# mormj/newsched

Measured on NVIDIA B200. Metric: Msamples/s FIR-ccf & FFT-4096 flowgraph at 1/2/4/8 B200; % of HBM/FP32 roofline, higher is better.
Workload: dtype f32

## Files before the change

newsched_b200/csrc/fft.cu:

```cuda
#include <cmath>
#include <cstdlib>
#include <vector>

#include "fft_core.cuh"

#ifndef B200_FFT_TW2
#define B200_FFT_TW2 1
#endif
#ifndef B200_FFT_SHFL
#define B200_FFT_SHFL 0
#endif
#ifndef B200_FFT_LATEBAR
#define B200_FFT_LATEBAR 0
#endif

namespace b200 {

template <bool FWD, int OUT>
__global__ void __launch_bounds__(256, 2)
    fft4096_kernel(const float2* __restrict__ in, void* __restrict__ out, long long n_vec,
                   const float* __restrict__ weff, const float2* __restrict__ tw1,
                   const float2* __restrict__ tw2)
{
    __shared__ float2 sA[16 * F4K_STRIDE];
    __shared__ float2 sT2[256];
    const int tid = threadIdx.x;

    float wreg[16];
    float2 t1[16];
#pragma unroll
    for (int i = 0; i < 16; i++) {
        wreg[i] = __ldg(weff + i * 256 + tid);
        t1[i] = __ldg(tw1 + i * 256 + tid);
    }
    sT2[tid] = __ldg(tw2 + tid);
    __syncthreads();

    for (long long vec = blockIdx.x; vec < n_vec; vec += gridDim.x) {
        const float2* x = in + vec * 4096;
        float2 v[16];
        if (tid == 0 && vec + gridDim.x < n_vec && ((uintptr_t)in % 16 == 0))
            asm volatile("cp.async.bulk.prefetch.L2.global [%0], %1;" ::"l"(in + (vec + gridDim.x) * 4096),
                         "r"(4096 * 8)
                         : "memory");
#pragma unroll
        for (int i = 0; i < 16; i++)
            v[i] = __ldcs(x + i * 256 + tid);
#pragma unroll
        for (int i = 0; i < 16; i++)
            v[i] = __fmul2_rn(v[i], make_float2(wreg[i], wreg[i]));
        dft16<FWD>(v);
#pragma unroll
        for (int k0 = 0; k0 < 16; k0++)
            sA[k0 * F4K_STRIDE + tid] = cmul(v[pos16(k0)], t1[k0]);
        __syncthreads();
        {
            const int k0 = tid >> 4, n0 = tid & 15;
            float2* row = sA + k0 * F4K_STRIDE + n0;
#pragma unroll
            for (int i = 0; i < 16; i++)
                v[i] = row[i * 16];
            dft16<FWD>(v);
            row[0] = v[pos16(0)];
#pragma unroll
            for (int k1 = 1; k1 < 16; k1++)
                row[k1 * 16] = cmul(v[pos16(k1)], sT2[k1 * 16 + n0]);
        }
        __syncthreads();
        {
            const int k0 = tid & 15, k1 = tid >> 4;
            const float2* row = sA + k0 * F4K_STRIDE + k1 * 16;
#pragma unroll
            for (int i = 0; i < 16; i++)
                v[i] = row[i];
            dft16<FWD>(v);
            if (OUT == B200_FFT_OUT_COMPLEX) {
                float2* y = reinterpret_cast<float2*>(out) + vec * 4096;
#pragma unroll
                for (int k2 = 0; k2 < 16; k2++)
                    __stcs(y + k2 * 256 + tid, v[pos16(k2)]);
            } else {
                float* y = reinterpret_cast<float*>(out) + vec * 4096;
#pragma unroll
                for (int k2 = 0; k2 < 16; k2++) {
                    float2 z = v[pos16(k2)];
                    float p = fmaf(z.x, z.x, z.y * z.y);
                    __stcs(y + k2 * 256 + tid, OUT == B200_FFT_OUT_MAG ? sqrt_approx(p) : p);
                }
            }
        }
        __syncthreads();
    }
}

#ifndef B200_FFT_DBUF
#define B200_FFT_DBUF 0
#endif
#ifndef F4K_NBUF_MAG
#define F4K_NBUF_MAG 2
#endif
constexpr int f4k_nbuf(int out) { return out == B200_FFT_OUT_COMPLEX ? 1 : F4K_NBUF_MAG; }
constexpr size_t f4k_tma_smem(int out)
{
    return (size_t)f4k_nbuf(out) * 4096 * 8 + (B200_FFT_DBUF ? 2 : 1) * 16 * F4K_STRIDE * 8 + 256 * 8 + 32;
}

template <bool FWD, int OUT>
__global__ void __launch_bounds__(256, 2)
    fft4096_tma_kernel(const float2* __restrict__ in, void* __restrict__ out, long long n_vec,
                       const float* __restrict__ weff, const float2* __restrict__ tw1,
                       const float2* __restrict__ tw2)
{
    constexpr int NBUF = f4k_nbuf(OUT);
    extern __shared__ __align__(128) unsigned char smem_raw[];
    float2* sIn0 = reinterpret_cast<float2*>(smem_raw);
    float2* sA0 = sIn0 + 4096 * NBUF;
#if B200_FFT_DBUF
    float2* sT2 = sA0 + 2 * 16 * F4K_STRIDE;
#else
    float2* sT2 = sA0 + 16 * F4K_STRIDE;
#endif
    uint64_t* bar0 = reinterpret_cast<uint64_t*>(sT2 + 256);
    const int tid = threadIdx.x;

    if (tid == 0) {
#pragma unroll
        for (int i = 0; i < NBUF; i++)
            mbar_init(bar0 + i, 1);
        fence_mbar_init();
    }
    float wreg[16];
    float2 t1[16];
#pragma unroll
    for (int i = 0; i < 16; i++) {
        wreg[i] = __ldg(weff + i * 256 + tid);
        t1[i] = __ldg(tw1 + i * 256 + tid);
    }
    sT2[tid] = __ldg(tw2 + tid);
    __syncthreads();
#if B200_FFT_TW2 == 1
    float2 t2r[16];
#pragma unroll
    for (int k1 = 1; k1 < 16; k1++)
        t2r[k1] = sT2[k1 * 16 + (tid & 15)];
#endif
    pdl_wait();
    pdl_launch_dependents();
    long long vec = blockIdx.x;
    if (tid == 0) {
#pragma unroll
        for (int i = 0; i < NBUF; i++)
            if (vec + (long long)i * gridDim.x < n_vec) {
                mbar_arrive_expect_tx(bar0 + i, 4096 * 8);
                bulk_copy_g2s(sIn0 + 4096 * i, in + (vec + (long long)i * gridDim.x) * 4096, 4096 * 8, bar0 + i);
            }
    }
    uint32_t phase = 0;
    int it = 0;
    for (; vec < n_vec; vec += gridDim.x, it++) {
        float2 v[16];
        float2* sIn = sIn0 + (NBUF == 2 ? (it & 1) * 4096 : 0);
        uint64_t* bar = bar0 + (NBUF == 2 ? (it & 1) : 0);
        const uint32_t par = NBUF == 2 ? (uint32_t)((it >> 1) & 1) : phase;
#if B200_FFT_DBUF
        float2* sA = sA0 + (phase ? 16 * F4K_STRIDE : 0);
#else
        float2* sA = sA0;
#endif
        mbar_wait(bar, par);
        phase ^= 1;
#pragma unroll
        for (int i = 0; i < 16; i++)
            v[i] = sIn[i * 256 + tid];
#pragma unroll
        for (int i = 0; i < 16; i++)
            v[i] = __fmul2_rn(v[i], make_float2(wreg[i], wreg[i]));
        dft16<FWD>(v);
#if B200_FFT_LATEBAR
        __syncthreads();
#endif
#pragma unroll
        for (int k0 = 0; k0 < 16; k0++)
            sA[k0 * F4K_STRIDE + tid] = cmul(v[pos16(k0)], t1[k0]);
#if B200_FFT_TW2 == 2
        float2 t2r[16];
#pragma unroll
        for (int k1 = 1; k1 < 16; k1++)
            t2r[k1] = sT2[k1 * 16 + (tid & 15)];
#endif
        __syncthreads();
        if (tid == 0 && vec + (long long)NBUF * gridDim.x < n_vec) {
            mbar_arrive_expect_tx(bar, 4096 * 8);
            bulk_copy_g2s(sIn, in + (vec + (long long)NBUF * gridDim.x) * 4096, 4096 * 8, bar);
        }
#if B200_FFT_SHFL
        {
            const int k0 = tid >> 4, n0 = tid & 15;
            const float2* row = sA + k0 * F4K_STRIDE + n0;
#pragma unroll
            for (int i = 0; i < 16; i++)
                v[i] = row[i * 16];
            dft16<FWD>(v);
            float2 w[16];
            w[0] = v[pos16(0)];
#pragma unroll
            for (int k1 = 1; k1 < 16; k1++)
                w[k1] = cmul(v[pos16(k1)], t2r[k1]);
#pragma unroll
            for (int sft = 1; sft < 16; sft <<= 1) {
                const bool up = (n0 & sft) != 0;
#pragma unroll
                for (int i = 0; i < 16; i++) {
                    if (i & sft)
                        continue;
                    const float2 send = up ? w[i] : w[i | sft];
                    float2 recv;
                    recv.x = __shfl_xor_sync(0xffffffffu, send.x, sft);
                    recv.y = __shfl_xor_sync(0xffffffffu, send.y, sft);
                    if (up)
                        w[i] = recv;
                    else
                        w[i | sft] = recv;
                }
            }
#pragma unroll
            for (int i = 0; i < 16; i++)
                v[i] = w[i];
            dft16<FWD>(v);
            const int k1 = n0;
            if (OUT == B200_FFT_OUT_COMPLEX) {
                float2* y = reinterpret_cast<float2*>(out) + vec * 4096;
#pragma unroll
                for (int k2 = 0; k2 < 16; k2++)
                    __stcs(y + k2 * 256 + k1 * 16 + k0, v[pos16(k2)]);
            } else {
                float* y = reinterpret_cast<float*>(out) + vec * 4096;
#pragma unroll
                for (int k2 = 0; k2 < 16; k2++) {
                    float2 z = v[pos16(k2)];
                    float p = fmaf(z.x, z.x, z.y * z.y);
                    __stcs(y + k2 * 256 + k1 * 16 + k0, OUT == B200_FFT_OUT_MAG ? sqrt_approx(p) : p);
                }
            }
        }
#else
        {
            const int k0 = tid >> 4, n0 = tid & 15;
            float2* row = sA + k0 * F4K_STRIDE + n0;
#pragma unroll
            for (int i = 0; i < 16; i++)
                v[i] = row[i * 16];
            dft16<FWD>(v);
            row[0] = v[pos16(0)];
#pragma unroll
            for (int k1 = 1; k1 < 16; k1++)
#if B200_FFT_TW2
                row[k1 * 16] = cmul(v[pos16(k1)], t2r[k1]);
#else
                row[k1 * 16] = cmul(v[pos16(k1)], sT2[k1 * 16 + n0]);
#endif
        }
        __syncthreads();
        {
            const int k0 = tid & 15, k1 = tid >> 4;
            const float2* row = sA + k0 * F4K_STRIDE + k1 * 16;
#pragma unroll
            for (int i = 0; i < 16; i++)
                v[i] = row[i];
            dft16<FWD>(v);
            if (OUT == B200_FFT_OUT_COMPLEX) {
                float2* y = reinterpret_cast<float2*>(out) + vec * 4096;
#pragma unroll
                for (int k2 = 0; k2 < 16; k2++)
                    __stcs(y + k2 * 256 + tid, v[pos16(k2)]);
            } else {
                float* y = reinterpret_cast<float*>(out) + vec * 4096;
#pragma unroll
                for (int k2 = 0; k2 < 16; k2++) {
                    float2 z = v[pos16(k2)];
                    float p = fmaf(z.x, z.x, z.y * z.y);
                    __stcs(y + k2 * 256 + tid, OUT == B200_FFT_OUT_MAG ? sqrt_approx(p) : p);
                }
            }
        }
#endif
#if !B200_FFT_LATEBAR && !B200_FFT_DBUF
        __syncthreads();
#endif
    }
}

#ifndef B200_F8K_EARLY
#define B200_F8K_EARLY 0
#endif
constexpr size_t F8K_SMEM = 8192 * 8 + 16 * F4K_STRIDE * 8 + 256 * 8 + 32;

template <bool FWD, int I>
__device__ __forceinline__ float2 mul_w32(float2 z)
{
    constexpr double kPi = 3.14159265358979323846;
    constexpr float cr[16] = { 1.f, 0.98078528040323043f, 0.92387953251128674f, 0.83146961230254524f,
                               0.70710678118654752f, 0.55557023301960218f, 0.38268343236508977f,
                               0.19509032201612825f, 0.f, -0.19509032201612825f, -0.38268343236508977f,
                               -0.55557023301960218f, -0.70710678118654752f, -0.83146961230254524f,
                               -0.92387953251128674f, -0.98078528040323043f };
    constexpr float si[16] = { 0.f, 0.19509032201612825f, 0.38268343236508977f, 0.55557023301960218f,
                               0.70710678118654752f, 0.83146961230254524f, 0.92387953251128674f,
                               0.98078528040323043f, 1.f, 0.98078528040323043f, 0.92387953251128674f,
                               0.83146961230254524f, 0.70710678118654752f, 0.55557023301960218f,
                               0.38268343236508977f, 0.19509032201612825f };
    (void)kPi;
    if (I == 0)
        return z;
    constexpr float wr = cr[I], wi = FWD ? -si[I] : si[I];
    return make_float2(fmaf(-z.y, wi, z.x * wr), fmaf(z.x, wi, z.y * wr));
}

template <bool FWD, int I = 0>
__device__ __forceinline__ void f8k_split(float2 (&a)[16], float2* sIn, const float* __restrict__ w0,
                                          const float* __restrict__ w1, float2 wt, int tid)
{
    if constexpr (I < 16) {
        const float2 x0 = __fmul2_rn(sIn[I * 256 + tid], make_float2(w0[I], w0[I]));
        const float2 x1 = __fmul2_rn(sIn[4096 + I * 256 + tid], make_float2(w1[I], w1[I]));
        a[I] = x0 + x1;
        sIn[I * 256 + tid] = cmul(mul_w32<FWD, I>(x0 - x1), wt);
        f8k_split<FWD, I + 1>(a, sIn, w0, w1, wt, tid);
    }
}

template <bool FWD, int OUT>
__global__ void __launch_bounds__(256, 2)
    fft8192_kernel(const float2* __restrict__ in, void* __restrict__ out, long long n_vec,
                   const float* __restrict__ weff, const float2* __restrict__ tw1,
                   const float2* __restrict__ tw2, float odd_sign)
{
    extern __shared__ __align__(128) unsigned char smem_raw[];
    float2* sIn = reinterpret_cast<float2*>(smem_raw);
    float2* sA = sIn + 8192;
    float2* sT2 = sA + 16 * F4K_STRIDE;
    uint64_t* bar = reinterpret_cast<uint64_t*>(sT2 + 256);
    const int tid = threadIdx.x;
    if (tid == 0) {
        mbar_init(bar, 1);
        mbar_init(bar + 1, 1);
        fence_mbar_init();
    }
    float2 t1[16];
#pragma unroll
    for (int i = 0; i < 16; i++)
        t1[i] = __ldg(tw1 + i * 256 + tid);
    sT2[tid] = __ldg(tw2 + tid);
    float2 wt;
    {
        float sn, cs_;
        sincospif((float)tid / 4096.0f, &sn, &cs_);
        wt = make_float2(cs_ * odd_sign, (FWD ? -sn : sn) * odd_sign);
    }
    __syncthreads();
    pdl_wait();
    pdl_launch_dependents();
    long long vec = blockIdx.x;
    if (tid == 0 && vec < n_vec) {
        mbar_arrive_expect_tx(bar, 4096 * 8);
        bulk_copy_g2s(sIn, in + vec * 8192, 4096 * 8, bar);
        mbar_arrive_expect_tx(bar + 1, 4096 * 8);
        bulk_copy_g2s(sIn + 4096, in + vec * 8192 + 4096, 4096 * 8, bar + 1);
    }
    uint32_t phase = 0;
    for (; vec < n_vec; vec += gridDim.x) {
        float2 e[16], v[16];
// ... 436 lines not shown
            __stcs(dst, make_float4(m[0], m[1], m[2], m[3]));
            __stcs(dst + 1, make_float4(m[4], m[5], m[6], m[7]));
        }
    }
}

template <bool FWD, int OUT>
__global__ void __launch_bounds__(512)
    fft_generic_kernel(const float2* __restrict__ in, void* __restrict__ out, long long n_vec, int N,
                       int log2n, int vpb, const float* __restrict__ weff,
                       const float2* __restrict__ tw, float2 post, int flip)
{
    extern __shared__ __align__(16) float2 sbuf[];
    const int per_cta = vpb * N;
    float2* bx = sbuf;
    float2* by = sbuf + per_cta;
    const long long v0 = (long long)blockIdx.x * vpb;
    const int nv = (int)((n_vec - v0) < vpb ? (n_vec - v0) : vpb);
    if (nv <= 0)
        return;
    const int tot = nv * N;
    const float2* x = in + v0 * N;
    for (int i = threadIdx.x; i < tot; i += blockDim.x) {
        float2 t = __ldcs(x + i);
        float w = __ldg(weff + (i & (N - 1)));
        bx[i] = make_float2(t.x * w, t.y * w);
    }
    __syncthreads();
    const int half = N >> 1;
    int s_log = 0;
    for (int n_log = log2n; n_log >= 1; n_log--, s_log++) {
        const int m = 1 << (n_log - 1);
        const int s = 1 << s_log;
        for (int i = threadIdx.x; i < nv * half; i += blockDim.x) {
            int vi = i / half;
            int bi = i - vi * half;
            int p = bi >> s_log;
            int q = bi & (s - 1);
            const float2* xb = bx + vi * N;
            float2* yb = by + vi * N;
            float2 a = xb[q + s * p];
            float2 b = xb[q + s * (p + m)];
            float2 w = __ldg(tw + (p << (log2n - n_log)));
            float2 d = a - b;
            yb[q + s * 2 * p] = a + b;
            yb[q + s * (2 * p + 1)] = cmul(d, w);
        }
        __syncthreads();
        float2* t = bx;
        bx = by;
        by = t;
    }
    for (int i = threadIdx.x; i < tot; i += blockDim.x) {
        float2 z = bx[i];
        int k = i & (N - 1);
        if (OUT == B200_FFT_OUT_COMPLEX) {
            z = cmul(z, post);
            if (flip && (k & 1))
                z = make_float2(-z.x, -z.y);
            __stcs(reinterpret_cast<float2*>(out) + v0 * N + i, z);
        } else {
            float pw = fmaf(z.x, z.x, z.y * z.y);
            __stcs(reinterpret_cast<float*>(out) + v0 * N + i,
                   OUT == B200_FFT_OUT_MAG ? sqrt_approx(pw) : pw);
        }
    }
}

}

using namespace b200;

struct b200_fft {
    int N = 0, log2n = 0;
    int forward = 1, out_mode = 0;
    int flip = 0;
    float2 post{ 1.f, 0.f };
    float* d_weff = nullptr;
    float2* d_tw1 = nullptr;
    float2* d_tw2 = nullptr;
    float2* d_tw = nullptr;
    int vpb = 1;
    int grid_4k = 296;
    int use_tma = 1;
};

template <bool FWD, int OUT>
static int fft_run_t(b200_fft* h, const void* d_in, void* d_out, long long n_vec, cudaStream_t s)
{
    if (h->N == 4096) {
        long long g = n_vec < h->grid_4k ? n_vec : h->grid_4k;
        if (h->use_tma && (uintptr_t)d_in % 16 == 0)
            B200_LAUNCH_PDL((fft4096_tma_kernel<FWD, OUT>), (unsigned)g, 256, f4k_tma_smem(OUT), s,
                        (const float2*)d_in, d_out, n_vec, h->d_weff, h->d_tw1, h->d_tw2);
        else
            B200_LAUNCH((fft4096_kernel<FWD, OUT>), (unsigned)g, 256, 0, s, (const float2*)d_in, d_out,
                        n_vec, h->d_weff, h->d_tw1, h->d_tw2);
    } else if (h->N == 16 || h->N == 32 || h->N == 64 || h->N == 128) {
        const int R0 = h->N / 16, V = 4096 / h->N;
        long long nb = (n_vec + V - 1) / V;
        long long g = nb < h->grid_4k ? nb : h->grid_4k;
        const int tma_ok = (uintptr_t)d_in % 16 == 0;
#define FFT_SM_GO(R)                                                                                     \
    B200_LAUNCH_PDL((fft_small_kernel<R, FWD, OUT>), (unsigned)g, 256, fsm<R>::SMEM, s, (const float2*)d_in, \
                d_out, n_vec, h->d_weff, h->d_tw1, h->flip, tma_ok)
        switch (R0) {
        case 1: FFT_SM_GO(1); break;
        case 2: FFT_SM_GO(2); break;
        case 4: FFT_SM_GO(4); break;
        default: FFT_SM_GO(8); break;
        }
#undef FFT_SM_GO
    } else if (h->N == 256 || h->N == 512 || h->N == 1024 || h->N == 2048) {
        const int R0 = h->N / 256, V = 16 / R0;
        long long nb = (n_vec + V - 1) / V;
        long long g = nb < h->grid_4k ? nb : h->grid_4k;
        const int tma_ok = (uintptr_t)d_in % 16 == 0;
#define FFT_R0_GO(R)                                                                                  \
    B200_LAUNCH_PDL((fft_r0_kernel<R, FWD, OUT>), (unsigned)g, 256, fr0<R>::SMEM, s, (const float2*)d_in, \
                d_out, n_vec, h->d_weff, h->d_tw1, h->d_tw2, tma_ok)
        switch (R0) {
        case 1: FFT_R0_GO(1); break;
        case 2: FFT_R0_GO(2); break;
        case 4: FFT_R0_GO(4); break;
        default: FFT_R0_GO(8); break;
        }
#undef FFT_R0_GO
    } else if (h->N == 8 && (uintptr_t)d_in % 16 == 0 && (uintptr_t)d_out % 16 == 0) {
        long long blocks = (n_vec + 255) / 256;
        const long long cap = 16LL * sm_count();
        B200_LAUNCH((fft8_kernel<FWD, OUT>), (unsigned)(blocks < cap ? blocks : cap), 256, 0, s, (const float2*)d_in,
                    d_out, n_vec, h->d_weff, h->post, h->flip);
    } else if (h->N == 8192 && h->d_tw1 && (uintptr_t)d_in % 16 == 0 && (uintptr_t)d_out % 16 == 0) {
        long long g = n_vec < h->grid_4k ? n_vec : h->grid_4k;
        B200_LAUNCH_PDL((fft8192_kernel<FWD, OUT>), (unsigned)g, 256, F8K_SMEM, s, (const float2*)d_in, d_out, n_vec,
                    h->d_weff, h->d_tw1, h->d_tw2, h->flip ? -1.f : 1.f);
    } else {
        long long blocks = (n_vec + h->vpb - 1) / h->vpb;
        if (blocks > 0x7fffffffLL)
            return set_err(B200_ERR_ARG, "fft: too many vectors for one call");
        int work = h->vpb * h->N / 2;
        int nt = work < 512 ? (work < 32 ? 32 : work) : 512;
        size_t smem = sizeof(float2) * 2 * (size_t)h->vpb * h->N;
        B200_LAUNCH((fft_generic_kernel<FWD, OUT>), (unsigned)blocks, nt, smem, s,
                    (const float2*)d_in, d_out, n_vec, h->N, h->log2n, h->vpb, h->d_weff, h->d_tw,
                    h->post, h->flip);
    }
    return B200_OK;
}

template <bool FWD>
static int fft_run_o(b200_fft* h, const void* d_in, void* d_out, long long n_vec, cudaStream_t s)
{
    switch (h->out_mode) {
    case B200_FFT_OUT_COMPLEX:
        return fft_run_t<FWD, B200_FFT_OUT_COMPLEX>(h, d_in, d_out, n_vec, s);
    case B200_FFT_OUT_MAG:
        return fft_run_t<FWD, B200_FFT_OUT_MAG>(h, d_in, d_out, n_vec, s);
    default:
        return fft_run_t<FWD, B200_FFT_OUT_MAG_SQUARED>(h, d_in, d_out, n_vec, s);
    }
}

template <bool FWD, int OUT>
static cudaError_t fft_tma_attr()
{
    return cudaFuncSetAttribute(fft4096_tma_kernel<FWD, OUT>,
                                cudaFuncAttributeMaxDynamicSharedMemorySize, (int)f4k_tma_smem(OUT));
}

template <int R0, bool FWD, int OUT>
static cudaError_t fft_r0_attr()
{
    return cudaFuncSetAttribute(fft_r0_kernel<R0, FWD, OUT>, cudaFuncAttributeMaxDynamicSharedMemorySize,
                                (int)fr0<R0>::SMEM);
}
template <int R0>
static cudaError_t fft_r0_attr_all()
{
    cudaError_t e = cudaSuccess;
    if ((e = fft_r0_attr<R0, true, 0>()) != cudaSuccess) return e;
    if ((e = fft_r0_attr<R0, true, 1>()) != cudaSuccess) return e;
    if ((e = fft_r0_attr<R0, true, 2>()) != cudaSuccess) return e;
    if ((e = fft_r0_attr<R0, false, 0>()) != cudaSuccess) return e;
    if ((e = fft_r0_attr<R0, false, 1>()) != cudaSuccess) return e;
    return fft_r0_attr<R0, false, 2>();
}

template <int R0, bool FWD, int OUT>
static cudaError_t fft_small_attr()
{
    return cudaFuncSetAttribute(fft_small_kernel<R0, FWD, OUT>, cudaFuncAttributeMaxDynamicSharedMemorySize,
                                (int)fsm<R0>::SMEM);
}
template <int R0>
static cudaError_t fft_small_attr_all()
{
    cudaError_t e = cudaSuccess;
    if ((e = fft_small_attr<R0, true, 0>()) != cudaSuccess) return e;
    if ((e = fft_small_attr<R0, true, 1>()) != cudaSuccess) return e;
    if ((e = fft_small_attr<R0, true, 2>()) != cudaSuccess) return e;
    if ((e = fft_small_attr<R0, false, 0>()) != cudaSuccess) return e;
    if ((e = fft_small_attr<R0, false, 1>()) != cudaSuccess) return e;
    return fft_small_attr<R0, false, 2>();
}

template <bool FWD, int OUT>
static cudaError_t fft_generic_attr()
{
    return cudaFuncSetAttribute(fft_generic_kernel<FWD, OUT>,
                                cudaFuncAttributeMaxDynamicSharedMemorySize, 160 * 1024);
}

extern "C" {

int b200_fft_destroy(b200_fft* h)
{
    if (!h)
        return B200_OK;
    cudaFree(h->d_weff);
    cudaFree(h->d_tw1);
    cudaFree(h->d_tw2);
    cudaFree(h->d_tw);
    delete h;
    return B200_OK;
}

int b200_fft_create(const b200_fft_params* p, b200_fft** out)
{
    if (!p || !out)
        return set_err(B200_ERR_ARG, "fft_create: null argument");
    *out = nullptr;
    const int N = p->n;
    if (N < 8 || N > 8192 || (N & (N - 1)))
        return set_err(B200_ERR_UNSUPPORTED, "fft_create: N must be a power of two in [8, 8192], got %d", N);
    if (p->output < 0 || p->output > 2)
        return set_err(B200_ERR_ARG, "fft_create: bad output mode %d", p->output);
    b200_fft* h = new b200_fft();
    h->N = N;
    while ((1 << h->log2n) < N)
        h->log2n++;
    h->forward = p->forward ? 1 : 0;
    h->out_mode = p->output;
    const double sgn = h->forward ? -1.0 : 1.0;

    double kmag = 1.0, kph_re = 1.0, kph_im = 0.0;
    if (p->fuse_pre_multiply_const) {
        kmag = std::hypot((double)p->k_re, (double)p->k_im);
        if (kmag > 0.0) {
            kph_re = p->k_re / kmag;
            kph_im = p->k_im / kmag;
        }
    }
    std::vector<float> weff(N);
    for (int n = 0; n < N; n++) {
        double w;
        if (!h->forward && p->shift) {
            w = p->window ? (double)p->window[(n + N - N / 2) % N] : 1.0;
        } else {
            w = p->window ? (double)p->window[n] : 1.0;
            if (h->forward && p->shift && (n & 1))
                w = -w;
        }
        weff[n] = (float)(w * kmag);
    }
    h->flip = (!h->forward && p->shift) ? 1 : 0;
    h->post = make_float2((float)kph_re, (float)kph_im);

#define FFT_CUDA(call)                                                                   \
    do {                                                                                 \
        cudaError_t e__ = (call);                                                        \
        if (e__ != cudaSuccess) {                                                        \
            b200_fft_destroy(h);                                                         \
            return set_err(e__ == cudaErrorMemoryAllocation ? B200_ERR_NOMEM : B200_ERR_CUDA, \
                           "fft_create: %s -> %s", #call, cudaGetErrorString(e__));      \
        }                                                                                \
    } while (0)

    FFT_CUDA(cudaMalloc(&h->d_weff, sizeof(float) * N));
    FFT_CUDA(cudaMemcpy(h->d_weff, weff.data(), sizeof(float) * N, cudaMemcpyHostToDevice));
    if (N == 4096) {
        std::vector<float2> t1(16 * 256), t2(256);
        for (int k0 = 0; k0 < 16; k0++)
            for (int L = 0; L < 256; L++) {
                double ang = sgn * 2.0 * M_PI * (double)((L * k0) % 4096) / 4096.0;
                double wr = std::cos(ang), wi = std::sin(ang);
                double pr = kph_re, pi = kph_im;
                if (h->flip && (k0 & 1)) {
                    pr = -pr;
                    pi = -pi;
                }
                t1[k0 * 256 + L] = make_float2((float)(wr * pr - wi * pi), (float)(wr * pi + wi * pr));
            }
        for (int k1 = 0; k1 < 16; k1++)
            for (int n0 = 0; n0 < 16; n0++) {
                double ang = sgn * 2.0 * M_PI * (double)(n0 * k1) / 256.0;
                t2[k1 * 16 + n0] = make_float2((float)std::cos(ang), (float)std::sin(ang));
            }
        FFT_CUDA(cudaMalloc(&h->d_tw1, sizeof(float2) * t1.size()));
        FFT_CUDA(cudaMemcpy(h->d_tw1, t1.data(), sizeof(float2) * t1.size(), cudaMemcpyHostToDevice));
        FFT_CUDA(cudaMalloc(&h->d_tw2, sizeof(float2) * t2.size()));
        FFT_CUDA(cudaMemcpy(h->d_tw2, t2.data(), sizeof(float2) * t2.size(), cudaMemcpyHostToDevice));
        h->grid_4k = 2 * sm_count();
        if (const char* e = getenv("B200_FFT_TMA"))
            h->use_tma = atoi(e);
        if (const char* e = getenv("B200_FFT_GRID_PER_SM"))
            h->grid_4k = atoi(e) * sm_count();
        FFT_CUDA((fft_tma_attr<true, 0>()));
        FFT_CUDA((fft_tma_attr<true, 1>()));
        FFT_CUDA((fft_tma_attr<true, 2>()));
        FFT_CUDA((fft_tma_attr<false, 0>()));
        FFT_CUDA((fft_tma_attr<false, 1>()));
        FFT_CUDA((fft_tma_attr<false, 2>()));
    } else if (N == 16 || N == 32 || N == 64 || N == 128) {
        const int R0 = N / 16;
        std::vector<float2> t1((size_t)R0 * 16);
        for (int k0 = 0; k0 < R0; k0++)
            for (int n0 = 0; n0 < 16; n0++) {
                double ang = sgn * 2.0 * M_PI * (double)(n0 * k0) / (double)N;
                double wr = std::cos(ang), wi = std::sin(ang);
                t1[(size_t)k0 * 16 + n0] =
                    make_float2((float)(wr * kph_re - wi * kph_im), (float)(wr * kph_im + wi * kph_re));
            }
        FFT_CUDA(cudaMalloc(&h->d_tw1, sizeof(float2) * 128));
        FFT_CUDA(cudaMemset(h->d_tw1, 0, sizeof(float2) * 128));
        FFT_CUDA(cudaMemcpy(h->d_tw1, t1.data(), sizeof(float2) * t1.size(), cudaMemcpyHostToDevice));
        h->grid_4k = 2 * sm_count();
        FFT_CUDA(fft_small_attr_all<1>());
        FFT_CUDA(fft_small_attr_all<2>());
        FFT_CUDA(fft_small_attr_all<4>());
        FFT_CUDA(fft_small_attr_all<8>());
    } else if (N == 256 || N == 512 || N == 1024 || N == 2048) {
        const int R0 = N / 256;
        std::vector<float2> t1((size_t)R0 * 256), t2(256);
        for (int k0 = 0; k0 < R0; k0++)
            for (int L = 0; L < 256; L++) {
                double ang = sgn * 2.0 * M_PI * (double)((L * k0) % N) / (double)N;
                double wr = std::cos(ang), wi = std::sin(ang);
                double pr = kph_re, pi = kph_im;
                if (h->flip && R0 > 1 && (k0 & 1)) {
                    pr = -pr;
                    pi = -pi;
                }
                t1[(size_t)k0 * 256 + L] = make_float2((float)(wr * pr - wi * pi), (float)(wr * pi + wi * pr));
            }
        for (int k1 = 0; k1 < 16; k1++)
            for (int n0 = 0; n0 < 16; n0++) {
                double ang = sgn * 2.0 * M_PI * (double)(n0 * k1) / 256.0;
                double f = (h->flip && R0 == 1 && (k1 & 1)) ? -1.0 : 1.0;
                t2[k1 * 16 + n0] = make_float2((float)(f * std::cos(ang)), (float)(f * std::sin(ang)));
            }
        FFT_CUDA(cudaMalloc(&h->d_tw1, sizeof(float2) * t1.size()));
        FFT_CUDA(cudaMemcpy(h->d_tw1, t1.data(), sizeof(float2) * t1.size(), cudaMemcpyHostToDevice));
        FFT_CUDA(cudaMalloc(&h->d_tw2, sizeof(float2) * t2.size()));
        FFT_CUDA(cudaMemcpy(h->d_tw2, t2.data(), sizeof(float2) * t2.size(), cudaMemcpyHostToDevice));
        h->grid_4k = 2 * sm_count();
        FFT_CUDA(fft_r0_attr_all<1>());
        FFT_CUDA(fft_r0_attr_all<2>());
        FFT_CUDA(fft_r0_attr_all<4>());
        FFT_CUDA(fft_r0_attr_all<8>());
    } else {
        std::vector<float2> tw(N / 2);
        for (int j = 0; j < N / 2; j++) {
            double ang = sgn * 2.0 * M_PI * (double)j / (double)N;
            tw[j] = make_float2((float)std::cos(ang), (float)std::sin(ang));
        }
        FFT_CUDA(cudaMalloc(&h->d_tw, sizeof(float2) * tw.size()));
        FFT_CUDA(cudaMemcpy(h->d_tw, tw.data(), sizeof(float2) * tw.size(), cudaMemcpyHostToDevice));
        h->vpb = N >= 1024 ? 1 : 1024 / N;
        FFT_CUDA((fft_generic_attr<true, 0>()));
        FFT_CUDA((fft_generic_attr<true, 1>()));
        FFT_CUDA((fft_generic_attr<true, 2>()));
        FFT_CUDA((fft_generic_attr<false, 0>()));
        FFT_CUDA((fft_generic_attr<false, 1>()));
        FFT_CUDA((fft_generic_attr<false, 2>()));
        if (N == 8192 && !getenv("B200_FFT_GENERIC")) {
            std::vector<float2> t1(16 * 256), t2(256);
            for (int k0 = 0; k0 < 16; k0++)
                for (int L = 0; L < 256; L++) {
                    double ang = sgn * 2.0 * M_PI * (double)((L * k0) % 4096) / 4096.0;
                    double wr = std::cos(ang), wi = std::sin(ang);
                    t1[k0 * 256 + L] =
                        make_float2((float)(wr * kph_re - wi * kph_im), (float)(wr * kph_im + wi * kph_re));
                }
            for (int k1 = 0; k1 < 16; k1++)
                for (int n0 = 0; n0 < 16; n0++) {
                    double ang = sgn * 2.0 * M_PI * (double)(n0 * k1) / 256.0;
                    t2[k1 * 16 + n0] = make_float2((float)std::cos(ang), (float)std::sin(ang));
                }
            FFT_CUDA(cudaMalloc(&h->d_tw1, sizeof(float2) * t1.size()));
            FFT_CUDA(cudaMemcpy(h->d_tw1, t1.data(), sizeof(float2) * t1.size(), cudaMemcpyHostToDevice));
            FFT_CUDA(cudaMalloc(&h->d_tw2, sizeof(float2) * t2.size()));
            FFT_CUDA(cudaMemcpy(h->d_tw2, t2.data(), sizeof(float2) * t2.size(), cudaMemcpyHostToDevice));
            h->grid_4k = 2 * sm_count();
#define F8K_ATTR(FW, O) \
    FFT_CUDA(cudaFuncSetAttribute(fft8192_kernel<FW, O>, cudaFuncAttributeMaxDynamicSharedMemorySize, (int)F8K_SMEM))
// ... 43 lines not shown
```

newsched_b200/csrc/tc_ptx.cuh:

```cuda
#pragma once
#include <cuda_bf16.h>

#include "common.cuh"

namespace b200 {

__device__ __forceinline__ uint8_t* tc_align1024(uint8_t* raw)
{
    return raw + ((1024u - (smem_u32(raw) & 1023u)) & 1023u);
}

__device__ __forceinline__ void tc_fence_before() { asm volatile("tcgen05.fence::before_thread_sync;" ::: "memory"); }
__device__ __forceinline__ void tc_fence_after() { asm volatile("tcgen05.fence::after_thread_sync;" ::: "memory"); }
__device__ __forceinline__ void tc_alloc(uint32_t* smem_dst, uint32_t ncols)
{
    asm volatile("tcgen05.alloc.cta_group::1.sync.aligned.shared::cta.b32 [%0], %1;" ::"r"(smem_u32(smem_dst)), "r"(ncols)
                 : "memory");
    asm volatile("tcgen05.relinquish_alloc_permit.cta_group::1.sync.aligned;" ::: "memory");
}
__device__ __forceinline__ void tc_dealloc(uint32_t taddr, uint32_t ncols)
{
    asm volatile("tcgen05.dealloc.cta_group::1.sync.aligned.b32 %0, %1;" ::"r"(taddr), "r"(ncols) : "memory");
}
__device__ __forceinline__ void tc_commit(uint64_t* bar)
{
    asm volatile("tcgen05.commit.cta_group::1.mbarrier::arrive::one.shared::cluster.b64 [%0];" ::"r"(smem_u32(bar))
                 : "memory");
}
__device__ __forceinline__ void tc_mma_bf16(uint32_t d_tmem, uint64_t adesc, uint64_t bdesc, uint32_t idesc,
                                            uint32_t accumulate)
{
    asm volatile("{\n"
                 ".reg .pred p;\n"
                 "setp.ne.b32 p, %4, 0;\n"
                 "tcgen05.mma.cta_group::1.kind::f16 [%0], %1, %2, %3, p;\n"
                 "}\n" ::"r"(d_tmem),
                 "l"(adesc), "l"(bdesc), "r"(idesc), "r"(accumulate)
                 : "memory");
}
__device__ __forceinline__ uint32_t tc_elect_one()
{
    uint32_t pred = 0, laneid = 0;
    asm volatile("{\n"
                 ".reg .b32 %%rx;\n"
                 ".reg .pred %%px;\n"
                 "elect.sync %%rx|%%px, %2;\n"
                 "@%%px mov.s32 %1, 1;\n"
                 "mov.s32 %0, %%rx;\n"
                 "}\n"
                 : "+r"(laneid), "+r"(pred)
                 : "r"(0xFFFFFFFFu));
    return pred;
}
__device__ __forceinline__ int tc_warp_idx() { return __shfl_sync(0xffffffffu, (int)(threadIdx.x >> 5), 0); }

__device__ __forceinline__ void tc_commit_w(uint32_t bar_saddr)
{
    asm volatile("{\n"
                 ".reg .pred e;\n"
                 "elect.sync _|e, 0xffffffff;\n"
                 "@e tcgen05.commit.cta_group::1.mbarrier::arrive::one.shared::cluster.b64 [%0];\n"
                 "}\n" ::"r"(bar_saddr)
                 : "memory");
}
__device__ __forceinline__ void tc_mma_bf16_w(uint32_t d_tmem, uint64_t adesc, uint64_t bdesc, uint32_t idesc,
                                              uint32_t accumulate)
{
    asm volatile("{\n"
                 ".reg .pred p, e;\n"
                 "setp.ne.b32 p, %4, 0;\n"
                 "elect.sync _|e, 0xffffffff;\n"
                 "@e tcgen05.mma.cta_group::1.kind::f16 [%0], %1, %2, %3, p;\n"
                 "}\n" ::"r"(d_tmem),
                 "l"(adesc), "l"(bdesc), "r"(idesc), "r"(accumulate)
                 : "memory");
}
__device__ __forceinline__ void tc_mma_bf16_ts_w(uint32_t d_tmem, uint32_t a_tmem, uint64_t bdesc, uint32_t idesc,
                                                 uint32_t accumulate)
{
    asm volatile("{\n"
                 ".reg .pred p, e;\n"
                 "setp.ne.b32 p, %4, 0;\n"
                 "elect.sync _|e, 0xffffffff;\n"
                 "@e tcgen05.mma.cta_group::1.kind::f16 [%0], [%1], %2, %3, p;\n"
                 "}\n" ::"r"(d_tmem),
                 "r"(a_tmem), "l"(bdesc), "r"(idesc), "r"(accumulate)
                 : "memory");
}
__device__ __forceinline__ void tc_ld32(uint32_t taddr, float (&v)[32])
{
    uint32_t* u = reinterpret_cast<uint32_t*>(v);
    asm volatile("tcgen05.ld.sync.aligned.32x32b.x32.b32 "
                 "{%0, %1, %2, %3, %4, %5, %6, %7, %8, %9, %10, %11, %12, %13, %14, %15, "
                 "%16, %17, %18, %19, %20, %21, %22, %23, %24, %25, %26, %27, %28, %29, %30, %31}, [%32];"
                 : "=r"(u[0]), "=r"(u[1]), "=r"(u[2]), "=r"(u[3]), "=r"(u[4]), "=r"(u[5]), "=r"(u[6]), "=r"(u[7]),
                   "=r"(u[8]), "=r"(u[9]), "=r"(u[10]), "=r"(u[11]), "=r"(u[12]), "=r"(u[13]), "=r"(u[14]), "=r"(u[15]),
                   "=r"(u[16]), "=r"(u[17]), "=r"(u[18]), "=r"(u[19]), "=r"(u[20]), "=r"(u[21]), "=r"(u[22]), "=r"(u[23]),
                   "=r"(u[24]), "=r"(u[25]), "=r"(u[26]), "=r"(u[27]), "=r"(u[28]), "=r"(u[29]), "=r"(u[30]), "=r"(u[31])
                 : "r"(taddr)
                 : "memory");
}
__device__ __forceinline__ void tc_wait_ld() { asm volatile("tcgen05.wait::ld.sync.aligned;" ::: "memory"); }

__device__ __forceinline__ uint64_t tc_desc(uint32_t saddr, int mode)
{
    uint64_t d = (uint64_t)((saddr >> 4) & 0x3FFF);
    d |= (uint64_t)1 << 16;
    d |= (uint64_t)(1024 >> 4) << 32;
    d |= (uint64_t)1 << 46;
    if (mode)
        d |= (uint64_t)((saddr >> 7) & 7) << 49;
    d |= (uint64_t)2 << 61;
    return d;
}

__device__ __forceinline__ uint32_t tc_plane_off(uint32_t i)
{
    return (i >> 6) * 128u + ((((i >> 3) & 7u) ^ ((i >> 6) & 7u)) << 4) + (i & 7u) * 2u;
}

__device__ __forceinline__ void tc_split(float v, __nv_bfloat16& hi, __nv_bfloat16& lo)
{
    hi = __float2bfloat16_rn(v);
    lo = __float2bfloat16_rn(v - __bfloat162float(hi));
}

__device__ __forceinline__ void tc_mma_bf16_ts(uint32_t d_tmem, uint32_t a_tmem, uint64_t bdesc, uint32_t idesc,
                                               uint32_t accumulate)
{
    asm volatile("{\n"
                 ".reg .pred p;\n"
                 "setp.ne.b32 p, %4, 0;\n"
                 "tcgen05.mma.cta_group::1.kind::f16 [%0], [%1], %2, %3, p;\n"
                 "}\n" ::"r"(d_tmem),
                 "r"(a_tmem), "l"(bdesc), "r"(idesc), "r"(accumulate)
                 : "memory");
}
__device__ __forceinline__ void tc_st8(uint32_t taddr, const uint32_t (&v)[8])
{
    asm volatile("tcgen05.st.sync.aligned.32x32b.x8.b32 [%0], {%1, %2, %3, %4, %5, %6, %7, %8};" ::"r"(taddr), "r"(v[0]),
                 "r"(v[1]), "r"(v[2]), "r"(v[3]), "r"(v[4]), "r"(v[5]), "r"(v[6]), "r"(v[7])
                 : "memory");
}

}
```

Measured before the change: 489,500.

## Stash FFT-4096 twiddles and window in tensor memory to raise occupancy

Moves the per-thread window weights and the stage-1 and stage-2 twiddles out of registers and shared memory into tensor memory (TMEM). The kernel now reloads them with tcgen05.ld each iteration, overlapping each load with the DFT work. This frees registers and removes the sT2 shared array, so launch bounds go from 2 to 3 blocks per SM and the magnitude path drops to single input buffering. The grid is sized from the occupancy query, and the shared-memory carveout is set to maximum. In exchange it adds TMEM load latency on every iteration, a TMEM alloc/dealloc per block, and removes the shuffle and late-barrier variants.

```diff
diff --git a/newsched_b200/csrc/fft.cu b/newsched_b200/csrc/fft.cu
--- a/newsched_b200/csrc/fft.cu
+++ b/newsched_b200/csrc/fft.cu
@@ -3,16 +3,7 @@
 #include <vector>
 
 #include "fft_core.cuh"
-
-#ifndef B200_FFT_TW2
-#define B200_FFT_TW2 1
-#endif
-#ifndef B200_FFT_SHFL
-#define B200_FFT_SHFL 0
-#endif
-#ifndef B200_FFT_LATEBAR
-#define B200_FFT_LATEBAR 0
-#endif
+#include "tc_ptx.cuh"
 
 namespace b200 {
 
@@ -93,20 +84,22 @@
     }
 }
 
-#ifndef B200_FFT_DBUF
-#define B200_FFT_DBUF 0
+constexpr int F4K_TMEM_COLS = 128;
+#ifndef F4K_NBUF_MAG
+#define F4K_NBUF_MAG 1
 #endif
-#ifndef F4K_NBUF_MAG
-#define F4K_NBUF_MAG 2
+#ifndef F4K_MINB_MAG
+#define F4K_MINB_MAG 3
+#endif
+#ifndef F4K_MINB_CPX
+#define F4K_MINB_CPX 3
 #endif
 constexpr int f4k_nbuf(int out) { return out == B200_FFT_OUT_COMPLEX ? 1 : F4K_NBUF_MAG; }
-constexpr size_t f4k_tma_smem(int out)
-{
-    return (size_t)f4k_nbuf(out) * 4096 * 8 + (B200_FFT_DBUF ? 2 : 1) * 16 * F4K_STRIDE * 8 + 256 * 8 + 32;
-}
+constexpr int f4k_min_blocks(int out) { return out == B200_FFT_OUT_COMPLEX ? F4K_MINB_CPX : F4K_MINB_MAG; }
+constexpr size_t f4k_tma_smem(int out) { return (size_t)f4k_nbuf(out) * 4096 * 8 + 16 * F4K_STRIDE * 8 + 32; }
 
 template <bool FWD, int OUT>
-__global__ void __launch_bounds__(256, 2)
+__global__ void __launch_bounds__(256, f4k_min_blocks(OUT))
     fft4096_tma_kernel(const float2* __restrict__ in, void* __restrict__ out, long long n_vec,
                        const float* __restrict__ weff, const float2* __restrict__ tw1,
                        const float2* __restrict__ tw2)
@@ -114,14 +107,10 @@
     constexpr int NBUF = f4k_nbuf(OUT);
     extern __shared__ __align__(128) unsigned char smem_raw[];
     float2* sIn0 = reinterpret_cast<float2*>(smem_raw);
-    float2* sA0 = sIn0 + 4096 * NBUF;
-#if B200_FFT_DBUF
-    float2* sT2 = sA0 + 2 * 16 * F4K_STRIDE;
-#else
-    float2* sT2 = sA0 + 16 * F4K_STRIDE;
-#endif
-    uint64_t* bar0 = reinterpret_cast<uint64_t*>(sT2 + 256);
-    const int tid = threadIdx.x;
+    float2* sA = sIn0 + 4096 * NBUF;
+    uint64_t* bar0 = reinterpret_cast<uint64_t*>(sA + 16 * F4K_STRIDE);
+    uint32_t* tmem_slot = reinterpret_cast<uint32_t*>(bar0 + NBUF);
+    const int tid = threadIdx.x, warp = tc_warp_idx();
 
     if (tid == 0) {
 #pragma unroll
@@ -129,21 +118,52 @@
             mbar_init(bar0 + i, 1);
         fence_mbar_init();
     }
-    float wreg[16];
-    float2 t1[16];
-#pragma unroll
-    for (int i = 0; i < 16; i++) {
-        wreg[i] = __ldg(weff + i * 256 + tid);
-        t1[i] = __ldg(tw1 + i * 256 + tid);
-    }
-    sT2[tid] = __ldg(tw2 + tid);
+    if (warp == 0) {
+        __syncwarp();
+        tc_alloc(tmem_slot, F4K_TMEM_COLS);
+    }
+    tc_fence_before();
     __syncthreads();
-#if B200_FFT_TW2 == 1
-    float2 t2r[16];
-#pragma unroll
-    for (int k1 = 1; k1 < 16; k1++)
-        t2r[k1] = sT2[k1 * 16 + (tid & 15)];
-#endif
+    tc_fence_after();
+    const uint32_t tl = *tmem_slot + ((uint32_t)((warp & 3) * 32) << 16);
+    const uint32_t tm_w = tl + (warp >> 2) * 48, tm_t1 = tm_w + 16, tm_t2 = tl + 96;
+    {
+        uint32_t u[8];
+#pragma unroll
+        for (int c = 0; c < 2; c++) {
+#pragma unroll
+            for (int j = 0; j < 8; j++)
+                u[j] = __float_as_uint(__ldg(weff + (c * 8 + j) * 256 + tid));
+            tc_st8(tm_w + c * 8, u);
+        }
+#pragma unroll
+        for (int c = 0; c < 4; c++) {
+#pragma unroll
+            for (int j = 0; j < 4; j++) {
+                const float2 t = __ldg(tw1 + (c * 4 + j) * 256 + tid);
+                u[2 * j] = __float_as_uint(t.x);
+                u[2 * j + 1] = __float_as_uint(t.y);
+            }
+            tc_st8(tm_t1 + c * 8, u);
+        }
+        if (warp < 4) {
+#pragma unroll
+            for (int c = 0; c < 4; c++) {
+#pragma unroll
+                for (int j = 0; j < 4; j++) {
+                    const int k1 = 1 + c * 4 + j;
+                    const float2 t = k1 < 16 ? __ldg(tw2 + k1 * 16 + (tid & 15)) : make_float2(0.f, 0.f);
+                    u[2 * j] = __float_as_uint(t.x);
+                    u[2 * j + 1] = __float_as_uint(t.y);
+                }
+                tc_st8(tm_t2 + c * 8, u);
+            }
+        }
+        asm volatile("tcgen05.wait::st.sync.aligned;" ::: "memory");
+    }
+    tc_fence_before();
+    __syncthreads();
+    tc_fence_after();
     pdl_wait();
     pdl_launch_dependents();
     long long vec = blockIdx.x;
@@ -159,106 +179,54 @@
     int it = 0;
     for (; vec < n_vec; vec += gridDim.x, it++) {
         float2 v[16];
+        float c[16], d[16];
         float2* sIn = sIn0 + (NBUF == 2 ? (it & 1) * 4096 : 0);
         uint64_t* bar = bar0 + (NBUF == 2 ? (it & 1) : 0);
         const uint32_t par = NBUF == 2 ? (uint32_t)((it >> 1) & 1) : phase;
-#if B200_FFT_DBUF
-        float2* sA = sA0 + (phase ? 16 * F4K_STRIDE : 0);
-#else
-        float2* sA = sA0;
-#endif
+        tc_ld16(tm_w, c);
         mbar_wait(bar, par);
         phase ^= 1;
 #pragma unroll
         for (int i = 0; i < 16; i++)
             v[i] = sIn[i * 256 + tid];
+        tc_wait_ld16(c);
 #pragma unroll
         for (int i = 0; i < 16; i++)
-            v[i] = __fmul2_rn(v[i], make_float2(wreg[i], wreg[i]));
+            v[i] = __fmul2_rn(v[i], make_float2(c[i], c[i]));
+        tc_ld16(tm_t1, c);
         dft16<FWD>(v);
-#if B200_FFT_LATEBAR
-        __syncthreads();
-#endif
-#pragma unroll
-        for (int k0 = 0; k0 < 16; k0++)
-            sA[k0 * F4K_STRIDE + tid] = cmul(v[pos16(k0)], t1[k0]);
-#if B200_FFT_TW2 == 2
-        float2 t2r[16];
-#pragma unroll
-        for (int k1 = 1; k1 < 16; k1++)
-            t2r[k1] = sT2[k1 * 16 + (tid & 15)];
-#endif
+        tc_wait_ld16(c);
+        tc_ld16(tm_t1 + 16, d);
+#pragma unroll
+        for (int k0 = 0; k0 < 8; k0++)
+            sA[k0 * F4K_STRIDE + tid] = cmul(v[pos16(k0)], make_float2(c[2 * k0], c[2 * k0 + 1]));
+        tc_wait_ld16(d);
+#pragma unroll
+        for (int k0 = 8; k0 < 16; k0++)
+            sA[k0 * F4K_STRIDE + tid] = cmul(v[pos16(k0)], make_float2(d[2 * k0 - 16], d[2 * k0 - 15]));
         __syncthreads();
         if (tid == 0 && vec + (long long)NBUF * gridDim.x < n_vec) {
             mbar_arrive_expect_tx(bar, 4096 * 8);
             bulk_copy_g2s(sIn, in + (vec + (long long)NBUF * gridDim.x) * 4096, 4096 * 8, bar);
         }
-#if B200_FFT_SHFL
-        {
-            const int k0 = tid >> 4, n0 = tid & 15;
-            const float2* row = sA + k0 * F4K_STRIDE + n0;
-#pragma unroll
-            for (int i = 0; i < 16; i++)
-                v[i] = row[i * 16];
-            dft16<FWD>(v);
-            float2 w[16];
-            w[0] = v[pos16(0)];
-#pragma unroll
-            for (int k1 = 1; k1 < 16; k1++)
-                w[k1] = cmul(v[pos16(k1)], t2r[k1]);
-#pragma unroll
-            for (int sft = 1; sft < 16; sft <<= 1) {
-                const bool up = (n0 & sft) != 0;
-#pragma unroll
-                for (int i = 0; i < 16; i++) {
-                    if (i & sft)
-                        continue;
-                    const float2 send = up ? w[i] : w[i | sft];
-                    float2 recv;
-                    recv.x = __shfl_xor_sync(0xffffffffu, send.x, sft);
-                    recv.y = __shfl_xor_sync(0xffffffffu, send.y, sft);
-                    if (up)
-                        w[i] = recv;
-                    else
-                        w[i | sft] = recv;
-                }
-            }
-#pragma unroll
-            for (int i = 0; i < 16; i++)
-                v[i] = w[i];
-            dft16<FWD>(v);
-            const int k1 = n0;
-            if (OUT == B200_FFT_OUT_COMPLEX) {
-                float2* y = reinterpret_cast<float2*>(out) + vec * 4096;
-#pragma unroll
-                for (int k2 = 0; k2 < 16; k2++)
-                    __stcs(y + k2 * 256 + k1 * 16 + k0, v[pos16(k2)]);
-            } else {
-                float* y = reinterpret_cast<float*>(out) + vec * 4096;
-#pragma unroll
-                for (int k2 = 0; k2 < 16; k2++) {
-                    float2 z = v[pos16(k2)];
-                    float p = fmaf(z.x, z.x, z.y * z.y);
-                    __stcs(y + k2 * 256 + k1 * 16 + k0, OUT == B200_FFT_OUT_MAG ? sqrt_approx(p) : p);
-                }
-            }
-        }
-#else
         {
             const int k0 = tid >> 4, n0 = tid & 15;
             float2* row = sA + k0 * F4K_STRIDE + n0;
 #pragma unroll
             for (int i = 0; i < 16; i++)
                 v[i] = row[i * 16];
+            tc_ld16(tm_t2, c);
             dft16<FWD>(v);
+            tc_wait_ld16(c);
+            tc_ld16(tm_t2 + 16, d);
             row[0] = v[pos16(0)];
 #pragma unroll
-            for (int k1 = 1; k1 < 16; k1++)
-#if B200_FFT_TW2
-                row[k1 * 16] = cmul(v[pos16(k1)], t2r[k1]);
-#else
-                row[k1 * 16] = cmul(v[pos16(k1)], sT2[k1 * 16 + n0]);
-#endif
+            for (int k1 = 1; k1 < 9; k1++)
+                row[k1 * 16] = cmul(v[pos16(k1)], make_float2(c[2 * k1 - 2], c[2 * k1 - 1]));
+            tc_wait_ld16(d);
+#pragma unroll
+            for (int k1 = 9; k1 < 16; k1++)
+                row[k1 * 16] = cmul(v[pos16(k1)], make_float2(d[2 * k1 - 18], d[2 * k1 - 17]));
         }
         __syncthreads();
         {
@@ -283,10 +251,13 @@
                 }
             }
         }
-#endif
-#if !B200_FFT_LATEBAR && !B200_FFT_DBUF
-        __syncthreads();
-#endif
+        __syncthreads();
+    }
+    tc_fence_before();
+    __syncthreads();
+    if (warp == 0) {
+        tc_fence_after();
+        tc_dealloc(*tmem_slot, F4K_TMEM_COLS);
     }
 }
 
@@ -889,6 +860,7 @@
     float2* d_tw = nullptr;
     int vpb = 1;
     int grid_4k = 296;
+    int grid_4k_tma = 296;
     int use_tma = 1;
 };
 
@@ -897,8 +869,9 @@
 {
     if (h->N == 4096) {
         long long g = n_vec < h->grid_4k ? n_vec : h->grid_4k;
+        long long gt = n_vec < h->grid_4k_tma ? n_vec : h->grid_4k_tma;
         if (h->use_tma && (uintptr_t)d_in % 16 == 0)
-            B200_LAUNCH_PDL((fft4096_tma_kernel<FWD, OUT>), (unsigned)g, 256, f4k_tma_smem(OUT), s,
+            B200_LAUNCH_PDL((fft4096_tma_kernel<FWD, OUT>), (unsigned)gt, 256, f4k_tma_smem(OUT), s,
                         (const float2*)d_in, d_out, n_vec, h->d_weff, h->d_tw1, h->d_tw2);
         else
             B200_LAUNCH((fft4096_kernel<FWD, OUT>), (unsigned)g, 256, 0, s, (const float2*)d_in, d_out,
@@ -972,8 +945,26 @@
 template <bool FWD, int OUT>
 static cudaError_t fft_tma_attr()
 {
+    cudaError_t e = cudaFuncSetAttribute(fft4096_tma_kernel<FWD, OUT>, cudaFuncAttributePreferredSharedMemoryCarveout,
+                                         (int)cudaSharedmemCarveoutMaxShared);
+    if (e != cudaSuccess)
+        return e;
     return cudaFuncSetAttribute(fft4096_tma_kernel<FWD, OUT>,
                                 cudaFuncAttributeMaxDynamicSharedMemorySize, (int)f4k_tma_smem(OUT));
+}
+template <bool FWD, int OUT>
+static cudaError_t fft_tma_blocks_per_sm(int* n)
+{
+    return cudaOccupancyMaxActiveBlocksPerMultiprocessor(n, fft4096_tma_kernel<FWD, OUT>, 256, f4k_tma_smem(OUT));
+}
+template <bool FWD>
+static cudaError_t fft_tma_blocks_per_sm_o(int out, int* n)
+{
+    switch (out) {
+    case B200_FFT_OUT_COMPLEX: return fft_tma_blocks_per_sm<FWD, B200_FFT_OUT_COMPLEX>(n);
+    case B200_FFT_OUT_MAG: return fft_tma_blocks_per_sm<FWD, B200_FFT_OUT_MAG>(n);
+    default: return fft_tma_blocks_per_sm<FWD, B200_FFT_OUT_MAG_SQUARED>(n);
+    }
 }
 
 template <int R0, bool FWD, int OUT>
@@ -1111,14 +1102,22 @@
         h->grid_4k = 2 * sm_count();
         if (const char* e = getenv("B200_FFT_TMA"))
             h->use_tma = atoi(e);
-        if (const char* e = getenv("B200_FFT_GRID_PER_SM"))
-            h->grid_4k = atoi(e) * sm_count();
         FFT_CUDA((fft_tma_attr<true, 0>()));
         FFT_CUDA((fft_tma_attr<true, 1>()));
         FFT_CUDA((fft_tma_attr<true, 2>()));
         FFT_CUDA((fft_tma_attr<false, 0>()));
         FFT_CUDA((fft_tma_attr<false, 1>()));
         FFT_CUDA((fft_tma_attr<false, 2>()));
+        int per_sm = 0;
+        FFT_CUDA(h->forward ? fft_tma_blocks_per_sm_o<true>(h->out_mode, &per_sm)
+                            : fft_tma_blocks_per_sm_o<false>(h->out_mode, &per_sm));
+        if (per_sm < 1) {
+            b200_fft_destroy(h);
+            return set_err(B200_ERR_CUDA, "fft_create: fft4096_tma_kernel does not fit on an SM");
+        }
+        h->grid_4k_tma = per_sm * sm_count();
+        if (const char* e = getenv("B200_FFT_GRID_PER_SM"))
+            h->grid_4k = h->grid_4k_tma = atoi(e) * sm_count();
     } else if (N == 16 || N == 32 || N == 64 || N == 128) {
         const int R0 = N / 16;
         std::vector<float2> t1((size_t)R0 * 16);
diff --git a/newsched_b200/csrc/tc_ptx.cuh b/newsched_b200/csrc/tc_ptx.cuh
--- a/newsched_b200/csrc/tc_ptx.cuh
+++ b/newsched_b200/csrc/tc_ptx.cuh
@@ -101,6 +101,23 @@
                  : "memory");
 }
 __device__ __forceinline__ void tc_wait_ld() { asm volatile("tcgen05.wait::ld.sync.aligned;" ::: "memory"); }
+__device__ __forceinline__ void tc_ld16(uint32_t taddr, float (&v)[16])
+{
+    asm volatile("tcgen05.ld.sync.aligned.32x32b.x16.b32 "
+                 "{%0, %1, %2, %3, %4, %5, %6, %7, %8, %9, %10, %11, %12, %13, %14, %15}, [%16];"
+                 : "=f"(v[0]), "=f"(v[1]), "=f"(v[2]), "=f"(v[3]), "=f"(v[4]), "=f"(v[5]), "=f"(v[6]), "=f"(v[7]),
+                   "=f"(v[8]), "=f"(v[9]), "=f"(v[10]), "=f"(v[11]), "=f"(v[12]), "=f"(v[13]), "=f"(v[14]), "=f"(v[15])
+                 : "r"(taddr)
+                 : "memory");
+}
+__device__ __forceinline__ void tc_wait_ld16(float (&v)[16])
+{
+    asm volatile("tcgen05.wait::ld.sync.aligned;"
+                 : "+f"(v[0]), "+f"(v[1]), "+f"(v[2]), "+f"(v[3]), "+f"(v[4]), "+f"(v[5]), "+f"(v[6]), "+f"(v[7]),
+                   "+f"(v[8]), "+f"(v[9]), "+f"(v[10]), "+f"(v[11]), "+f"(v[12]), "+f"(v[13]), "+f"(v[14]), "+f"(v[15])
+                 :
+                 : "memory");
+}
 
 __device__ __forceinline__ uint64_t tc_desc(uint32_t saddr, int mode)
 {
```

After: 386,400, median of 6. -21.1%, worse.

## Compute FFT-4096 in place in TMA input tiles with ring buffering and swizzle

Applied to the files above, without the earlier changes.

Drops the separate padded shared-memory scratch array. The three FFT passes now run in place in the TMA landing tile, and the tiles rotate as a ring (2 for complex output, 3 for magnitude/power). An XOR swizzle on the middle-pass stores lets the final pass read 16-byte float4 segments without bank conflicts, and the trailing per-iteration __syncthreads is removed. The goal is to cut shared-memory footprint and barriers and to prefetch deeper. The cost is that correctness now depends on the async-proxy fence and the ring-slot reuse ordering. The experimental SHFL, LATEBAR and DBUF variants are removed.

```diff
diff --git a/newsched_b200/csrc/fft.cu b/newsched_b200/csrc/fft.cu
--- a/newsched_b200/csrc/fft.cu
+++ b/newsched_b200/csrc/fft.cu
@@ -6,12 +6,6 @@
 
 #ifndef B200_FFT_TW2
 #define B200_FFT_TW2 1
-#endif
-#ifndef B200_FFT_SHFL
-#define B200_FFT_SHFL 0
-#endif
-#ifndef B200_FFT_LATEBAR
-#define B200_FFT_LATEBAR 0
 #endif
 
 namespace b200 {
@@ -93,17 +87,10 @@
     }
 }
 
-#ifndef B200_FFT_DBUF
-#define B200_FFT_DBUF 0
-#endif
-#ifndef F4K_NBUF_MAG
-#define F4K_NBUF_MAG 2
-#endif
-constexpr int f4k_nbuf(int out) { return out == B200_FFT_OUT_COMPLEX ? 1 : F4K_NBUF_MAG; }
-constexpr size_t f4k_tma_smem(int out)
-{
-    return (size_t)f4k_nbuf(out) * 4096 * 8 + (B200_FFT_DBUF ? 2 : 1) * 16 * F4K_STRIDE * 8 + 256 * 8 + 32;
-}
+constexpr int f4k_ntile(int out) { return out == B200_FFT_OUT_COMPLEX ? 2 : 3; }
+constexpr size_t f4k_tma_smem(int out) { return (size_t)f4k_ntile(out) * (4096 * 8 + 8) + 256 * 8; }
+
+__device__ __forceinline__ int f4k_swz(int n0, int k0) { return (((n0 >> 1) ^ (k0 & 7)) << 1) | (n0 & 1); }
 
 template <bool FWD, int OUT>
 __global__ void __launch_bounds__(256, 2)
@@ -111,21 +98,16 @@
                        const float* __restrict__ weff, const float2* __restrict__ tw1,
                        const float2* __restrict__ tw2)
 {
-    constexpr int NBUF = f4k_nbuf(OUT);
+    constexpr int NT = f4k_ntile(OUT);
     extern __shared__ __align__(128) unsigned char smem_raw[];
-    float2* sIn0 = reinterpret_cast<float2*>(smem_raw);
-    float2* sA0 = sIn0 + 4096 * NBUF;
-#if B200_FFT_DBUF
-    float2* sT2 = sA0 + 2 * 16 * F4K_STRIDE;
-#else
-    float2* sT2 = sA0 + 16 * F4K_STRIDE;
-#endif
+    float2* sTile0 = reinterpret_cast<float2*>(smem_raw);
+    float2* sT2 = sTile0 + 4096 * NT;
     uint64_t* bar0 = reinterpret_cast<uint64_t*>(sT2 + 256);
     const int tid = threadIdx.x;
 
     if (tid == 0) {
 #pragma unroll
-        for (int i = 0; i < NBUF; i++)
+        for (int i = 0; i < NT; i++)
             mbar_init(bar0 + i, 1);
         fence_mbar_init();
     }
@@ -149,39 +131,28 @@
     long long vec = blockIdx.x;
     if (tid == 0) {
 #pragma unroll
-        for (int i = 0; i < NBUF; i++)
+        for (int i = 0; i < NT - 1; i++)
             if (vec + (long long)i * gridDim.x < n_vec) {
                 mbar_arrive_expect_tx(bar0 + i, 4096 * 8);
-                bulk_copy_g2s(sIn0 + 4096 * i, in + (vec + (long long)i * gridDim.x) * 4096, 4096 * 8, bar0 + i);
-            }
-    }
-    uint32_t phase = 0;
-    int it = 0;
-    for (; vec < n_vec; vec += gridDim.x, it++) {
+                bulk_copy_g2s(sTile0 + 4096 * i, in + (vec + (long long)i * gridDim.x) * 4096, 4096 * 8, bar0 + i);
+            }
+    }
+    int t = 0;
+    uint32_t par = 0;
+    for (; vec < n_vec; vec += gridDim.x) {
         float2 v[16];
-        float2* sIn = sIn0 + (NBUF == 2 ? (it & 1) * 4096 : 0);
-        uint64_t* bar = bar0 + (NBUF == 2 ? (it & 1) : 0);
-        const uint32_t par = NBUF == 2 ? (uint32_t)((it >> 1) & 1) : phase;
-#if B200_FFT_DBUF
-        float2* sA = sA0 + (phase ? 16 * F4K_STRIDE : 0);
-#else
-        float2* sA = sA0;
-#endif
-        mbar_wait(bar, par);
-        phase ^= 1;
+        float2* tile = sTile0 + t * 4096;
+        mbar_wait(bar0 + t, par);
 #pragma unroll
         for (int i = 0; i < 16; i++)
-            v[i] = sIn[i * 256 + tid];
+            v[i] = tile[i * 256 + tid];
 #pragma unroll
         for (int i = 0; i < 16; i++)
             v[i] = __fmul2_rn(v[i], make_float2(wreg[i], wreg[i]));
         dft16<FWD>(v);
-#if B200_FFT_LATEBAR
-        __syncthreads();
-#endif
 #pragma unroll
         for (int k0 = 0; k0 < 16; k0++)
-            sA[k0 * F4K_STRIDE + tid] = cmul(v[pos16(k0)], t1[k0]);
+            tile[k0 * 256 + tid] = cmul(v[pos16(k0)], t1[k0]);
 #if B200_FFT_TW2 == 2
         float2 t2r[16];
 #pragma unroll
@@ -189,84 +160,41 @@
             t2r[k1] = sT2[k1 * 16 + (tid & 15)];
 #endif
         __syncthreads();
-        if (tid == 0 && vec + (long long)NBUF * gridDim.x < n_vec) {
-            mbar_arrive_expect_tx(bar, 4096 * 8);
-            bulk_copy_g2s(sIn, in + (vec + (long long)NBUF * gridDim.x) * 4096, 4096 * 8, bar);
-        }
-#if B200_FFT_SHFL
+        const int tn = t == 0 ? NT - 1 : t - 1;
+        if (tid == 0 && vec + (long long)(NT - 1) * gridDim.x < n_vec) {
+            fence_proxy_async();
+            mbar_arrive_expect_tx(bar0 + tn, 4096 * 8);
+            bulk_copy_g2s(sTile0 + tn * 4096, in + (vec + (long long)(NT - 1) * gridDim.x) * 4096, 4096 * 8,
+                          bar0 + tn);
+        }
         {
             const int k0 = tid >> 4, n0 = tid & 15;
-            const float2* row = sA + k0 * F4K_STRIDE + n0;
+            float2* row = tile + k0 * 256;
 #pragma unroll
             for (int i = 0; i < 16; i++)
-                v[i] = row[i * 16];
+                v[i] = row[i * 16 + n0];
+            __syncwarp();
             dft16<FWD>(v);
-            float2 w[16];
-            w[0] = v[pos16(0)];
-#pragma unroll
-            for (int k1 = 1; k1 < 16; k1++)
-                w[k1] = cmul(v[pos16(k1)], t2r[k1]);
-#pragma unroll
-            for (int sft = 1; sft < 16; sft <<= 1) {
-                const bool up = (n0 & sft) != 0;
-#pragma unroll
-                for (int i = 0; i < 16; i++) {
-                    if (i & sft)
-                        continue;
-                    const float2 send = up ? w[i] : w[i | sft];
-                    float2 recv;
-                    recv.x = __shfl_xor_sync(0xffffffffu, send.x, sft);
-                    recv.y = __shfl_xor_sync(0xffffffffu, send.y, sft);
-                    if (up)
-                        w[i] = recv;
-                    else
-                        w[i | sft] = recv;
-                }
-            }
-#pragma unroll
-            for (int i = 0; i < 16; i++)
-                v[i] = w[i];
-            dft16<FWD>(v);
-            const int k1 = n0;
-            if (OUT == B200_FFT_OUT_COMPLEX) {
-                float2* y = reinterpret_cast<float2*>(out) + vec * 4096;
-#pragma unroll
-                for (int k2 = 0; k2 < 16; k2++)
-                    __stcs(y + k2 * 256 + k1 * 16 + k0, v[pos16(k2)]);
-            } else {
-                float* y = reinterpret_cast<float*>(out) + vec * 4096;
-#pragma unroll
-                for (int k2 = 0; k2 < 16; k2++) {
-                    float2 z = v[pos16(k2)];
-                    float p = fmaf(z.x, z.x, z.y * z.y);
-                    __stcs(y + k2 * 256 + k1 * 16 + k0, OUT == B200_FFT_OUT_MAG ? sqrt_approx(p) : p);
-                }
-            }
-        }
-#else
-        {
-            const int k0 = tid >> 4, n0 = tid & 15;
-            float2* row = sA + k0 * F4K_STRIDE + n0;
-#pragma unroll
-            for (int i = 0; i < 16; i++)
-                v[i] = row[i * 16];
-            dft16<FWD>(v);
-            row[0] = v[pos16(0)];
+            float2* dst = row + f4k_swz(n0, k0);
+            dst[0] = v[pos16(0)];
 #pragma unroll
             for (int k1 = 1; k1 < 16; k1++)
 #if B200_FFT_TW2
-                row[k1 * 16] = cmul(v[pos16(k1)], t2r[k1]);
+                dst[k1 * 16] = cmul(v[pos16(k1)], t2r[k1]);
 #else
-                row[k1 * 16] = cmul(v[pos16(k1)], sT2[k1 * 16 + n0]);
+                dst[k1 * 16] = cmul(v[pos16(k1)], sT2[k1 * 16 + n0]);
 #endif
         }
         __syncthreads();
         {
-            const int k0 = tid & 15, k1 = tid >> 4;
-            const float2* row = sA + k0 * F4K_STRIDE + k1 * 16;
-#pragma unroll
-            for (int i = 0; i < 16; i++)
-                v[i] = row[i];
+            const int k0 = tid & 15, k1 = tid >> 4, s = k0 & 7;
+            const float4* seg = reinterpret_cast<const float4*>(tile + k0 * 256 + k1 * 16);
+#pragma unroll
+            for (int j = 0; j < 8; j++) {
+                const float4 q = seg[j ^ s];
+                v[2 * j] = make_float2(q.x, q.y);
+                v[2 * j + 1] = make_float2(q.z, q.w);
+            }
             dft16<FWD>(v);
             if (OUT == B200_FFT_OUT_COMPLEX) {
                 float2* y = reinterpret_cast<float2*>(out) + vec * 4096;
@@ -283,10 +211,10 @@
                 }
             }
         }
-#endif
-#if !B200_FFT_LATEBAR && !B200_FFT_DBUF
-        __syncthreads();
-#endif
+        if (++t == NT) {
+            t = 0;
+            par ^= 1;
+        }
     }
 }
 
```

New measurement: 489,800 before, 511,500 after, median of 6. 4.4% higher.
